# alpc91/SGRL

Measured on AMD Instinct MI355X. Metric: env-steps/sec (whole node) + SET-actor fwd us/step, 3d_walker mix @8192 envs/GPU, higher is better.
Workload: dtype f64 (dynamics) / f32 (SET actor, obs); 1 GPU; 3D_Walker++ 8 variants x 1024 envs per GPU (config 3), random U(-1,1) actions, auto-reset, SET actor forward on every step, random-init weights; envs_per_gpu=8192, obs_max_len=287, action_max_len=21, replay_gather=none (single rank)

## Files before the change

include/sgrl_model.h:

```cpp
#ifndef SGRL_MODEL_H
#define SGRL_MODEL_H

#include <stdint.h>

#ifdef __HIPCC__
#define SGRL_HD __host__ __device__ inline
#else
#define SGRL_HD static inline
#endif

#define SGRL_MAGIC 0x5347524C
#define SGRL_MAXDEPTH 8

enum {
  SGRL_H_MAGIC = 0,
  SGRL_H_NBODY,
  SGRL_H_NJNT,
  SGRL_H_NQ,
  SGRL_H_NV,
  SGRL_H_NU,
  SGRL_H_NGEOM,
  SGRL_H_NPAIR,
  SGRL_H_INTEGRATOR,
  SGRL_H_FRAME_SKIP,
  SGRL_H_DONE_RULE,
  SGRL_H_TARGET_V2,
  SGRL_H_RESET_VEL_NORMAL,
  SGRL_H_NHEIGHT_BODIES,
  SGRL_H_HEIGHT_BODY0,
  SGRL_H_HEIGHT_BODY1,
  SGRL_H_MAX_ROWS,
  SGRL_H_PGS_ITERS,
  SGRL_H_SOLVER,
  SGRL_NHDR = 24
};

enum {
  SGRL_F_TIMESTEP = 0,
  SGRL_F_GRAV_X, SGRL_F_GRAV_Y, SGRL_F_GRAV_Z,
  SGRL_F_HEIGHT_LO, SGRL_F_HEIGHT_HI, SGRL_F_ANG_LIMIT,
  SGRL_F_ALIVE_BONUS, SGRL_F_HEADING_WEIGHT, SGRL_F_CTRL_COST,
  SGRL_F_RESET_POS_NOISE, SGRL_F_RESET_VEL_NOISE,
  SGRL_F_PGS_TOL,
  SGRL_F_TOTAL_MASS,
  SGRL_NFHDR = 16
};

enum { SGRL_GEOM_PLANE = 0, SGRL_GEOM_SPHERE = 2, SGRL_GEOM_CAPSULE = 3 };
enum { SGRL_JNT_FREE = 0, SGRL_JNT_HINGE = 3 };

#ifndef SGRL_CONST_AS
#define SGRL_CONST_AS
#endif
#ifndef SGRL_ITAB_AS
#define SGRL_ITAB_AS
#endif
#ifndef SGRL_FTAB_AS
#define SGRL_FTAB_AS
#endif
typedef const SGRL_CONST_AS int32_t* sgrl_hdr_t;
typedef const SGRL_CONST_AS double* sgrl_fhdr_t;
typedef const SGRL_ITAB_AS int32_t* sgrl_itab_t;
typedef const SGRL_FTAB_AS double* sgrl_ftab_t;

typedef struct SgrlModelView {
  sgrl_hdr_t hdr;
  sgrl_fhdr_t fhdr;
  int nbody, njnt, nq, nv, nu, ngeom, npair;
  sgrl_itab_t body_parent, body_jntadr, body_jntnum, body_dofadr, body_dofnum, body_limbtype;
  sgrl_itab_t jnt_type, jnt_body, jnt_qposadr, jnt_dofadr, jnt_limited;
  sgrl_itab_t dof_body, dof_jnt, dof_parent;
  sgrl_itab_t geom_type, geom_body;
  sgrl_itab_t pair_g1, pair_g2, pair_condim;
  sgrl_itab_t act_dof, act_slot;
  sgrl_itab_t body_depth;
  sgrl_itab_t body_path;
  sgrl_itab_t body_subend;
  sgrl_itab_t body_dofmask;
  sgrl_itab_t dof_act;
  sgrl_ftab_t qpos0;
  sgrl_ftab_t body_pos, body_quat, body_ipos, body_inertia, body_mass, body_invweight0;
  sgrl_ftab_t jnt_pos, jnt_axis, jnt_range, jnt_stiffness, jnt_solref, jnt_solimp, jnt_margin;
  sgrl_ftab_t dof_armature, dof_damping, dof_invweight0;
  sgrl_ftab_t geom_pos, geom_quat, geom_size;
  sgrl_ftab_t pair_mu, pair_margin, pair_solref, pair_solimp;
  sgrl_ftab_t act_gear, act_ctrlrange;
  int n_int, n_f64;
} SgrlModelView;

SGRL_HD int sgrl_model_view_dims(const int32_t* dims, sgrl_hdr_t hdr_src, sgrl_fhdr_t fhdr_src, sgrl_itab_t ib, sgrl_ftab_t fb,
                                 SgrlModelView* v) {
  if (dims[SGRL_H_MAGIC] != SGRL_MAGIC) return -1;
  v->hdr = hdr_src;
  v->fhdr = fhdr_src;
  const int nb = dims[SGRL_H_NBODY], nj = dims[SGRL_H_NJNT], nq = dims[SGRL_H_NQ], nv = dims[SGRL_H_NV];
  const int nu = dims[SGRL_H_NU], ng = dims[SGRL_H_NGEOM], np = dims[SGRL_H_NPAIR];
  v->nbody = nb; v->njnt = nj; v->nq = nq; v->nv = nv; v->nu = nu; v->ngeom = ng; v->npair = np;
  sgrl_itab_t p = ib + SGRL_NHDR;
  v->body_parent = p; p += nb;
  v->body_jntadr = p; p += nb;
  v->body_jntnum = p; p += nb;
  v->body_dofadr = p; p += nb;
  v->body_dofnum = p; p += nb;
  v->body_limbtype = p; p += nb;
  v->jnt_type = p; p += nj;
  v->jnt_body = p; p += nj;
  v->jnt_qposadr = p; p += nj;
  v->jnt_dofadr = p; p += nj;
  v->jnt_limited = p; p += nj;
  v->dof_body = p; p += nv;
  v->dof_jnt = p; p += nv;
  v->dof_parent = p; p += nv;
  v->geom_type = p; p += ng;
  v->geom_body = p; p += ng;
  v->pair_g1 = p; p += np;
  v->pair_g2 = p; p += np;
  v->pair_condim = p; p += np;
  v->act_dof = p; p += nu;
  v->act_slot = p; p += nu;
  v->body_depth = p; p += nb;
  v->body_path = p; p += 8 * nb;
  v->body_subend = p; p += nb;
  v->body_dofmask = p; p += 2 * nb;
  v->dof_act = p; p += nv;
  v->n_int = (int)(p - ib);
  sgrl_ftab_t f = fb + SGRL_NFHDR;
  v->qpos0 = f; f += nq;
  v->body_pos = f; f += 3 * nb;
  v->body_quat = f; f += 4 * nb;
  v->body_ipos = f; f += 3 * nb;
  v->body_inertia = f; f += 6 * nb;
  v->body_mass = f; f += nb;
  v->body_invweight0 = f; f += 2 * nb;
  v->jnt_pos = f; f += 3 * nj;
  v->jnt_axis = f; f += 3 * nj;
  v->jnt_range = f; f += 2 * nj;
  v->jnt_stiffness = f; f += nj;
  v->jnt_solref = f; f += 2 * nj;
  v->jnt_solimp = f; f += 5 * nj;
  v->jnt_margin = f; f += nj;
  v->dof_armature = f; f += nv;
  v->dof_damping = f; f += nv;
  v->dof_invweight0 = f; f += nv;
  v->geom_pos = f; f += 3 * ng;
  v->geom_quat = f; f += 4 * ng;
  v->geom_size = f; f += 3 * ng;
  v->pair_mu = f; f += np;
  v->pair_margin = f; f += np;
  v->pair_solref = f; f += 2 * np;
  v->pair_solimp = f; f += 5 * np;
  v->act_gear = f; f += nu;
  v->act_ctrlrange = f; f += 2 * nu;
  v->n_f64 = (int)(f - fb);
  return 0;
}

SGRL_HD int sgrl_model_view_from(sgrl_hdr_t hdr_src, sgrl_fhdr_t fhdr_src, sgrl_itab_t ib, sgrl_ftab_t fb,
                                 SgrlModelView* v) {
  int32_t dims[SGRL_NHDR];
  for (int k = 0; k < SGRL_NHDR; k++) dims[k] = hdr_src[k];
  return sgrl_model_view_dims(dims, hdr_src, fhdr_src, ib, fb, v);
}

SGRL_HD void sgrl_model_blob_sizes(const int32_t* hdr, int* n_int, int* n_f64) {
  const int nb = hdr[SGRL_H_NBODY], nj = hdr[SGRL_H_NJNT], nq = hdr[SGRL_H_NQ], nv = hdr[SGRL_H_NV];
  const int nu = hdr[SGRL_H_NU], ng = hdr[SGRL_H_NGEOM], np = hdr[SGRL_H_NPAIR];
  *n_int = SGRL_NHDR + 18 * nb + 5 * nj + 4 * nv + 2 * ng + 3 * np + 2 * nu;
  *n_f64 = SGRL_NFHDR + nq + 19 * nb + 17 * nj + 3 * nv + 10 * ng + 9 * np + 3 * nu;
}

SGRL_HD int sgrl_model_view(const int32_t* ib, const double* fb, SgrlModelView* v) {
  return sgrl_model_view_from((sgrl_hdr_t)ib, (sgrl_fhdr_t)fb, (sgrl_itab_t)ib, (sgrl_ftab_t)fb, v);
}


#endif
```

sgrl_amd/csrc/engine.hip:

```cpp
#include <hip/hip_runtime.h>

#include <algorithm>
#include <cmath>
#include <cstdio>
#include <cstdlib>
#include <cstring>
#include <string>
#include <vector>

#include "engine_kernel.h"
#include "stream_pick.h"

namespace {

thread_local std::string g_err;

int fail(int code, const std::string& msg) {
  g_err = msg;
  return code;
}
#define HIP_TRY(expr)                                                                              \
  do {                                                                                             \
    hipError_t _e = (expr);                                                                        \
    if (_e != hipSuccess)                                                                          \
// ... 360 lines not shown
  std::vector<int32_t> env_morph;
  std::vector<MorphDev> morphs(n_morph);
  e->d_ib.assign(n_morph, nullptr);
  e->d_fb.assign(n_morph, nullptr);
  int rc = SGRL_OK;
  for (int k = 0; k < n_morph && rc == SGRL_OK; k++) {
    SgrlModelView v;
    if (!ib[k] || !fb[k] || ib_len[k] < SGRL_NHDR || sgrl_model_view(ib[k], fb[k], &v) != 0) { rc = fail(SGRL_ERR_MODEL, "bad magic in model blob " + std::to_string(k)); break; }
    if (v.n_int != ib_len[k] || v.n_f64 != fb_len[k]) { rc = fail(SGRL_ERR_MODEL, "model blob " + std::to_string(k) + " has unexpected length"); break; }
    if (v.nv > 64 || v.nbody > 64 || v.npair > 64) { rc = fail(SGRL_ERR_LIMIT, "morphology exceeds 64 dofs/bodies/pairs"); break; }
    if ((v.nv | 1) > sgrl::kSlabLdy || ib[k][SGRL_H_MAX_ROWS] > sgrl::kSlabRows) { rc = fail(SGRL_ERR_LIMIT, "morphology exceeds the HBM constraint slab (nv <= 46, max_rows <= 256)"); break; }
    e->scratch_stride = std::max(e->scratch_stride, sgrl::slab_doubles(ib[k][SGRL_H_MAX_ROWS], v.nv | 1));
    e->max_geoms = std::max(e->max_geoms, v.ngeom);
    const int L = v.nbody - 1;
    if (41 * L > obs_max_len || 3 * L > action_max_len) { rc = fail(SGRL_ERR_ARG, "obs_max_len/action_max_len too small for morphology " + std::to_string(k)); break; }
    if (morph_count[k] < 0) { rc = fail(SGRL_ERR_ARG, "negative morph_count"); break; }
    sgrl::Layout o;
    sgrl::make_layout(ib[k], &o, v.n_int, SGRL_STAGE_FLOATS ? v.n_f64 : 0);
    if (17 * v.njnt + 7 * v.nbody > (o.lrows + 1) * o.ldy || 6 * v.nv > (o.lrows + 1) * o.ldy) {
      rc = fail(SGRL_ERR_LIMIT, "model " + std::to_string(k) + ": the constraint-row block is too small for the kinematics scratch (17 njnt + 7 nbody doubles)");
      break;
    }
    const int bytes = sgrl::layout_bytes(&o);
    if (bytes > 160 * 1024) { rc = fail(SGRL_ERR_LIMIT, "per-environment LDS slab exceeds 160 KiB"); break; }
    if (bytes > e->lds_bytes) e->lds_bytes = bytes;
    e->morph_lds.push_back(bytes);
    const int need = v.nq + v.nv + 4;
    if (need > e->stride) e->stride = need;
    for (int i = 0; i < morph_count[k]; i++) env_morph.push_back(k);
    if (hipMalloc(&e->d_ib[k], sizeof(int32_t) * ib_len[k]) != hipSuccess || hipMalloc(&e->d_fb[k], sizeof(double) * fb_len[k]) != hipSuccess) { rc = fail(SGRL_ERR_HIP, "hipMalloc(model) failed"); break; }
    (void)hipMemcpy(e->d_ib[k], ib[k], sizeof(int32_t) * ib_len[k], hipMemcpyHostToDevice);
    (void)hipMemcpy(e->d_fb[k], fb[k], sizeof(double) * fb_len[k], hipMemcpyHostToDevice);
    morphs[k].ib = e->d_ib[k];
    morphs[k].fb = e->d_fb[k];
    morphs[k].slot = -1;
    morphs[k].pad_ = 0;
  }
  if (rc == SGRL_OK && env_morph.empty()) rc = fail(SGRL_ERR_ARG, "no environments requested");
  if (rc != SGRL_OK) { sgrl_engine_destroy(e); return rc; }
  e->n_env = (int)env_morph.size();
  e->stride = (e->stride + 1) & ~1;
  bool ok = hipMalloc(&e->d_morphs, sizeof(MorphDev) * n_morph) == hipSuccess &&
            hipMalloc(&e->d_env_morph, sizeof(int32_t) * e->n_env) == hipSuccess &&
            hipMalloc(&e->d_block_env, sizeof(int32_t) * e->n_env) == hipSuccess &&
            hipMalloc(&e->d_step_env, sizeof(int32_t) * e->n_env) == hipSuccess &&
            hipMalloc(&e->d_step_mate, sizeof(int32_t) * e->n_env) == hipSuccess &&
            hipMalloc(&e->d_rec, sizeof(double) * (size_t)e->n_env * e->stride) == hipSuccess &&
            hipMalloc(&e->d_cnt, sizeof(int32_t) * (size_t)e->n_env * 4) == hipSuccess &&
            hipMalloc(&e->d_scratch, sizeof(double) * (size_t)e->n_env * e->scratch_stride) == hipSuccess &&
            hipMalloc(&e->d_cam_dist, sizeof(double) * n_morph) == hipSuccess;
  if (!ok) { sgrl_engine_destroy(e); return fail(SGRL_ERR_HIP, "hipMalloc(state) failed"); }
  e->cam_dist.assign(n_morph, std::nan(""));
  (void)hipMemset(e->d_cam_dist, 0, sizeof(double) * n_morph);
  (void)hipMemcpy(e->d_morphs, morphs.data(), sizeof(MorphDev) * n_morph, hipMemcpyHostToDevice);
  (void)hipMemcpy(e->d_env_morph, env_morph.data(), sizeof(int32_t) * e->n_env, hipMemcpyHostToDevice);
  {
    std::vector<int32_t> order(e->n_env);
    for (int i = 0; i < e->n_env; i++) order[i] = i;
    std::vector<int> spec(n_morph, -1);
    std::vector<int> pair_lds(n_morph, 0);
    std::vector<int> spec_lds(n_morph, 0);
    bool use_specs = false;
    {
      const char* sm = getenv("SGRL_SPECS");
      constexpr int kMaxSpecGroups = 4;
      if (!(sm && sm[0] == '0') && kNumMembers > 0) {
        bool all_light = true, all = true;
        for (int k = 0; k < n_morph; k++) if (morph_count[k] > 0) all_light = all_light && spec_for(ib[k], 4) >= 0;
        const char* pe = getenv("SGRL_PAIR");
        auto pair_bytes = [&](int k) -> int {
          const int m2 = spec_for(ib[k], 2);
          if (m2 < 0 || !kMembers[m2].dims[11] || (pe && pe[0] == '0')) return 0;
          SgrlModelView v;
          (void)sgrl_model_view(ib[k], fb[k], &v);
          sgrl::Layout po;
          sgrl::make_layout(ib[k], &po, v.n_int, 0, true);
          const int pb = sgrl::layout_bytes(&po);
          const bool scratch_ok = 17 * v.njnt + 7 * v.nbody <= (po.lrows + 1) * po.ldy && 6 * v.nv <= (po.lrows + 1) * po.ldy &&
                                  10 * v.nbody <= (po.lrows + 1) * po.ldy && v.nv <= 15;
          return (sgrl::workgroups_per_cu(pb) >= 8 && scratch_ok) ? pb : 0;
        };
        if (all_light) {
          bool all_pair = true;
          for (int k = 0; k < n_morph; k++) if (morph_count[k] > 0) all_pair = all_pair && morph_count[k] >= 2 && pair_bytes(k) > 0;
          if (all_pair) all_light = false;
        }
        std::vector<int> distinct;
        for (int k = 0; k < n_morph; k++) {
          if (morph_count[k] == 0) continue;
          int mb = spec_for(ib[k], all_light ? 4 : 2);
          all = all && mb >= 0;
          if (mb < 0) continue;
          spec[k] = kMembers[mb].family;
          morphs[k].slot = kMembers[mb].slot;
          spec_lds[k] = e->morph_lds[k];
          if (kFamilies[spec[k]].itab_global) {
            SgrlModelView v;
            (void)sgrl_model_view(ib[k], fb[k], &v);
            sgrl::Layout so;
            sgrl::make_layout(ib[k], &so, 0, SGRL_STAGE_FLOATS ? v.n_f64 : 0);
            if (17 * v.njnt + 7 * v.nbody <= (so.lrows + 1) * so.ldy && 6 * v.nv <= (so.lrows + 1) * so.ldy) spec_lds[k] = sgrl::layout_bytes(&so);
            else all = false;
          }
          if (kMembers[mb].dims[11]) pair_lds[k] = pair_bytes(k);
          if (std::find(distinct.begin(), distinct.end(), spec[k]) == distinct.end()) distinct.push_back(spec[k]);
        }
// ... 275 lines not shown
```

sgrl_amd/csrc/step_body.h:

```cpp
#pragma once

#include <math.h>
#include <stdint.h>

#include "../../include/sgrl_model.h"

#ifdef __HIPCC__
#define SGRL_DEV __device__ __forceinline__
#else
#define SGRL_DEV inline
#endif

namespace sgrl {

constexpr double kMinVal = 1e-15;
constexpr double kMinImp = 0.0001;
constexpr double kMaxImp = 0.9999;
constexpr double kPi = 3.14159265358979323846;
constexpr int kNAMax = 32;
constexpr int kBppMaxIter = 40;
constexpr int kSlabRows = 256;
constexpr int kPivotRows = 64;
constexpr int kPrevRows = 48;
constexpr int kSlabLdy = 47;
// ... 471 lines not shown
      ld6(cd, S + o.cdof + 6 * i);
      inert_mul(buf, ci, cd);
      S[o.L + tri(i) + i] = dot6(cd, buf) + m.dof_armature[i];
      for (int j = m.dof_parent[i]; j >= 0; j = m.dof_parent[j]) {
        double cj[6];
        ld6(cj, S + o.cdof + 6 * j);
        S[o.L + tri(i) + j] = dot6(cj, buf);
      }
    });
    if (W::hdr_const(m, SGRL_H_INTEGRATOR) == 0) {
      if (o.mfull_hbm) {
        double* const mh = big_scratch + slab_rows_doubles(o.maxrows, o.ldy);
        const int nt = nv * (nv + 1) / 2;
        w.lanes(64, [&](int l) { for (int k = l; k < nt; k += 64) mh[k] = S[o.L + k]; });
      } else {
        w.lanes(nv, [&](int i) { for (int k = 0; k <= i; k++) S[o.Mfull + tri(i) + k] = S[o.L + tri(i) + k]; });
      }
    }
    SGRL_TICK(2);
    linv = w.chol_inv_packed(nv, S + o.L, kMinVal);
    if (!linv) cholesky(o.L);
    SGRL_TICK(8);
  }

  SGRL_DEV void cholesky(int base) {
    const int nv = o.nv;
    for (int j = 0; j < nv - 1; j++) {
      double pj = S[base + tri(j) + j];
      if (pj < kMinVal) pj = kMinVal;
      const double wj = 1.0 / pj;
      const int sdim = nv - j - 1;
      w.lanes(sdim * (sdim + 1) / 2, [&](int p) {
        int a, b;
        tri_decode(p, &a, &b);
        const int i = j + 1 + a, k = j + 1 + b;
        S[base + tri(i) + k] -= S[base + tri(i) + j] * S[base + tri(k) + j] * wj;
      });
    }
    w.lanes(nv, [&](int j) {
      double pj = S[base + tri(j) + j];
      if (pj < kMinVal) pj = kMinVal;
      S[o.dinv + j] = sqrt(1.0 / pj);
    });
    w.lanes(nv * (nv - 1) / 2, [&](int p) {
      int a, b;
      tri_decode(p, &a, &b);
      S[base + tri(a + 1) + b] *= S[o.dinv + b];
    });
  }

  SGRL_DEV void solve_upper_inplace(int base, int xo) { w.trsv_upper(o.nv, S + base, S + o.dinv, S + xo); }
  SGRL_DEV void solve_lower_inplace(int base, int xo) { w.trsv_lower(o.nv, S + base, S + o.dinv, S + xo); }

  SGRL_DEV void geom_pose(int g, double* pos, double* mat) {
    const int b = m.geom_body[g];
    double t[3], gp[3], gq[4], gm[9], xm[9];
    ld3(gp, m.geom_pos + 3 * g);
    for (int k = 0; k < 9; k++) xm[k] = S[o.xmat + 9 * b + k];
    mat_vec(t, xm, gp);
    for (int k = 0; k < 3; k++) pos[k] = S[o.xpos + 3 * b + k] + t[k];
    for (int k = 0; k < 4; k++) gq[k] = m.geom_quat[4 * g + k];
    quat2mat(gm, gq);
    for (int r = 0; r < 3; r++)
      for (int c = 0; c < 3; c++) mat[3 * r + c] = xm[3 * r] * gm[c] + xm[3 * r + 1] * gm[3 + c] + xm[3 * r + 2] * gm[6 + c];
  }
  SGRL_DEV void make_frame(double* fr) {
    const double n2 = sqrt(dot3(fr + 3, fr + 3));
    if (n2 < 0.5) {
      fr[3] = 0; fr[4] = 0; fr[5] = 0;
      if (fr[1] < 0.5 && fr[1] > -0.5) fr[4] = 1; else fr[5] = 1;
    }
    const double d = dot3(fr, fr + 3);
    for (int k = 0; k < 3; k++) fr[3 + k] -= d * fr[k];
    const double n = sqrt(dot3(fr + 3, fr + 3));
    if (n < kMinVal) { fr[3] = 1; fr[4] = 0; fr[5] = 0; }
    else for (int k = 0; k < 3; k++) fr[3 + k] /= n;
    cross3(fr + 6, fr, fr + 3);
  }
  SGRL_DEV void put_contact(int slot, bool valid, double dist, const double* pos, const double* normal, const double* tangent) {
    I[o.con_valid + slot] = valid ? 1 : 0;
    if (!valid) return;
    double fr[9];
    for (int k = 0; k < 3; k++) { fr[k] = normal[k]; fr[3 + k] = tangent ? tangent[k] : 0.0; }
    make_frame(fr);
    S[o.con_dist + slot] = dist;
    for (int k = 0; k < 3; k++) S[o.con_pos + 3 * slot + k] = pos[k];
    for (int k = 0; k < 6; k++) S[o.con_frame + o.fstride * slot + k] = fr[k];
  }
  SGRL_DEV void plane_sphere(int slot, double margin, const double* ppos, const double* n, const double* c, double r, const double* tangent) {
    const double d[3] = {c[0] - ppos[0], c[1] - ppos[1], c[2] - ppos[2]};
    const double dist = dot3(d, n) - r;
    double pos[3];
    for (int k = 0; k < 3; k++) pos[k] = c[k] - n[k] * (r + 0.5 * dist);
    put_contact(slot, dist < margin, dist, pos, n, tangent);
  }
  SGRL_DEV void collide() {
    w.lanes(o.np, [&](int p) {
      const int g1 = m.pair_g1[p], g2 = m.pair_g2[p];
      double p1[3], m1[9], p2[3], m2[9];
      geom_pose(g1, p1, m1); geom_pose(g2, p2, m2);
      const double margin = m.pair_margin[p];
      const int t1 = m.geom_type[g1], t2 = m.geom_type[g2];
      if (t1 == SGRL_GEOM_PLANE) {
        const double n[3] = {m1[2], m1[5], m1[8]};
        if (t2 == SGRL_GEOM_SPHERE) {
          plane_sphere(2 * p, margin, p1, n, p2, m.geom_size[3 * g2], nullptr);
          I[o.con_valid + 2 * p + 1] = 0;
        } else {
          const double ax[3] = {m2[2], m2[5], m2[8]};
          const double h = m.geom_size[3 * g2 + 1], r = m.geom_size[3 * g2];
          double ca[3], cb[3];
          for (int k = 0; k < 3; k++) { ca[k] = p2[k] + ax[k] * h; cb[k] = p2[k] - ax[k] * h; }
          plane_sphere(2 * p, margin, p1, n, ca, r, ax);
          plane_sphere(2 * p + 1, margin, p1, n, cb, r, ax);
        }
      } else {
        const double a1[3] = {m1[2], m1[5], m1[8]}, a2[3] = {m2[2], m2[5], m2[8]};
        const double h1 = m.geom_size[3 * g1 + 1], h2 = m.geom_size[3 * g2 + 1];
        const double r1 = m.geom_size[3 * g1], r2 = m.geom_size[3 * g2];
        const double d[3] = {p1[0] - p2[0], p1[1] - p2[1], p1[2] - p2[2]};
        const double bb = dot3(a1, a2), c = dot3(a1, d), f = dot3(a2, d);
        const double den = 1.0 - bb * bb;
        const bool general = fabs(den) >= kMinVal;
        int made = 0;
        I[o.con_valid + 2 * p] = 0;
        I[o.con_valid + 2 * p + 1] = 0;
        for (int q = 0; q < (general ? 1 : 4) && made < 2; q++) {
          double s, t;
          if (general) {
            s = (bb * f - c) / den;
            if (s > h1) s = h1;
            if (s < -h1) s = -h1;
            t = bb * s + f;
            if (t > h2) { t = h2; s = bb * t - c; if (s > h1) s = h1; if (s < -h1) s = -h1; }
            else if (t < -h2) { t = -h2; s = bb * t - c; if (s > h1) s = h1; if (s < -h1) s = -h1; }
          } else if (q < 2) {
            s = q ? -h1 : h1; t = bb * s + f;
            if (t > h2) t = h2;
            if (t < -h2) t = -h2;
          } else {
            t = (q & 1) ? -h2 : h2; s = bb * t - c;
            if (s > h1) s = h1;
            if (s < -h1) s = -h1;
          }
          double c1[3], nn[3];
          for (int k = 0; k < 3; k++) { c1[k] = p1[k] + s * a1[k]; nn[k] = (p2[k] + t * a2[k]) - c1[k]; }
          const double len = sqrt(dot3(nn, nn));
          const double dist = len - r1 - r2;
          if (dist >= margin) continue;
          if (len < kMinVal) { nn[0] = 1; nn[1] = 0; nn[2] = 0; } else for (int k = 0; k < 3; k++) nn[k] /= len;
          double pos[3];
          for (int k = 0; k < 3; k++) pos[k] = c1[k] + nn[k] * (r1 + 0.5 * dist);
          put_contact(2 * p + made, true, dist, pos, nn, nullptr);
          made++;
        }
      }
    });
  }

  SGRL_DEV void bias_and_smooth_force() {
    w.lanes(o.nb, [&](int b) {
      if (b == 0) { for (int k = 0; k < 6; k++) S[o.cfrc + k] = 0; return; }
      double cv[6] = {0, 0, 0, 0, 0, 0};
      double ca[6] = {0, 0, 0, -m.fhdr[SGRL_F_GRAV_X], -m.fhdr[SGRL_F_GRAV_Y], -m.fhdr[SGRL_F_GRAV_Z]};
      const int depth = m.body_depth[b];
      for (int lvl = 0; lvl < depth; lvl++) {
        const int c = m.body_path[8 * b + lvl];
        const int j0 = m.body_jntadr[c], jn = m.body_jntnum[c];
        for (int j = j0; j < j0 + jn; j++) {
          const int d0 = m.jnt_dofadr[j];
// ... 5 lines not shown
            double cd[3][6], dd[6];
            for (int d = 0; d < 3; d++) ld6(cd[d], S + o.cdof + 6 * (d0 + 3 + d));
            for (int d = 0; d < 3; d++) {
              cross_motion(dd, cv, cd[d]);
              const double qv = S[o.qvel + d0 + 3 + d];
              for (int k = 0; k < 6; k++) ca[k] += dd[k] * qv;
            }
            for (int d = 0; d < 3; d++) {
              const double qv = S[o.qvel + d0 + 3 + d];
              for (int k = 0; k < 6; k++) cv[k] += cd[d][k] * qv;
            }
          } else {
            double cd[6], dd[6];
            ld6(cd, S + o.cdof + 6 * d0);
            cross_motion(dd, cv, cd);
            const double qv = S[o.qvel + d0];
            for (int k = 0; k < 6; k++) { ca[k] += dd[k] * qv; cv[k] += cd[k] * qv; }
          }
        }
      }
      double ci[10], f1[6], iv[6], f2[6];
      for (int k = 0; k < 10; k++) ci[k] = S[o.cinert + 10 * b + k];
      inert_mul(f1, ci, ca);
      inert_mul(iv, ci, cv);
      cross_force(f2, cv, iv);
      for (int k = 0; k < 6; k++) S[o.cfrc + 6 * b + k] = f1[k] + f2[k];
    });
    w.lanes(o.nv, [&](int d) {
      const int b = m.dof_body[d], e = m.body_subend[b];
      double f[6] = {0, 0, 0, 0, 0, 0}, cd[6];
      for (int c = b; c < e; c++)
        for (int k = 0; k < 6; k++) f[k] += S[o.cfrc + 6 * c + k];
      ld6(cd, S + o.cdof + 6 * d);
      const double bias = dot6(cd, f);
      const int j = m.dof_jnt[d];
      double passive = -m.dof_damping[d] * S[o.qvel + d];
      if (m.jnt_type[j] == SGRL_JNT_HINGE) {
        const int qa = m.jnt_qposadr[j];
        passive -= m.jnt_stiffness[j] * (S[o.qpos + qa] - m.qpos0[qa]);
      }
      double q = passive - bias;
      const int u = m.dof_act[d];
      if (u >= 0) {
        double c = S[o.ctrl + u];
        const double lo = m.act_ctrlrange[2 * u], hi = m.act_ctrlrange[2 * u + 1];
        if (c < lo) c = lo;
        if (c > hi) c = hi;
        q += m.act_gear[u] * c;
      }
      S[o.qfs + d] = q;
    });
  }

  SGRL_DEV double impedance(const double* solimp, double x_raw) {
    double dmin = solimp[0], dmax = solimp[1], width = solimp[2], mid = solimp[3], power = solimp[4];
    if (dmin < kMinImp) dmin = kMinImp;
    if (dmin > kMaxImp) dmin = kMaxImp;
    if (dmax < kMinImp) dmax = kMinImp;
    if (dmax > kMaxImp) dmax = kMaxImp;
    if (width < 0) width = 0;
    if (mid < kMinImp) mid = kMinImp;
    if (mid > kMaxImp) mid = kMaxImp;
    if (power < 1) power = 1;
    if (dmin == dmax || width <= kMinVal) return 0.5 * (dmin + dmax);
    const double x = fabs(x_raw) / width;
    if (x >= 1) return dmax;
    if (x <= 0) return dmin;
    double y;
    if (power == 1) y = x;
    else if (power == 2) y = (x <= mid) ? (x * x) / mid : 1 - ((1 - x) * (1 - x)) / (1 - mid);
    else if (x <= mid) y = pow(x, power) / pow(mid, power - 1);
    else y = 1 - pow(1 - x, power) / pow(1 - mid, power - 1);
    return dmin + y * (dmax - dmin);
  }
  SGRL_DEV void kb(const double* solref, const double* solimp, double* K, double* B) {
    double dmax = solimp[1];
    if (dmax < kMinImp) dmax = kMinImp;
    if (dmax > kMaxImp) dmax = kMaxImp;
    double tc = solref[0];
    const double dr = solref[1], h2 = 2 * m.fhdr[SGRL_F_TIMESTEP];
    if (tc < h2) tc = h2;
    *K = 1.0 / (dmax * dmax * tc * tc * dr * dr);
    *B = 2.0 / (dmax * tc);
  }

  struct Rows {
    double *Y, *eR, *earef, *eb, *ef, *eidg, *C;
    int32_t *kind, *src, *sub, *flist;
  };
  SGRL_DEV Rows rows_lds() const {
    return Rows{S + o.Y, S + o.eR, S + o.earef, S + o.eb, S + o.ef, S + o.eidg, S + o.dead,
                I + o.row_kind, I + o.row_src, I + o.row_sub, I + o.flist};
  }
  SGRL_DEV Rows rows_hbm() const {
    double* p = big_scratch;
    const int mr = o.maxrows;
    Rows r;
    r.C = p; p += kPivotRows * (kPivotRows + 1) / 2;
    r.Y = p; p += (mr + 1) * o.ldy;
    r.eR = p; p += mr; r.earef = p; p += mr; r.eb = p; p += mr; r.ef = p; p += mr;
    r.eidg = p; p += mr;
    int32_t* q = reinterpret_cast<int32_t*>(p);
    r.kind = q; r.src = q + mr; r.sub = q + 2 * mr; r.flist = q + 3 * mr;
    return r;
  }

  SGRL_DEV int count_rows() {
    const int nitem = 2 * o.nj + o.ncon;
    w.lanes(nitem, [&](int t) {
      int c = 0;
      if (t < 2 * o.nj) {
        const int j = t >> 1, side = (t & 1) ? 1 : -1;
        if (m.jnt_limited[j]) {
          const double q = S[o.qpos + m.jnt_qposadr[j]];
          const double dist = side * (m.jnt_range[2 * j + (side + 1) / 2] - q);
          if (dist < m.jnt_margin[j]) c = 1;
        }
      } else {
        const int sl = t - 2 * o.nj;
        if (I[o.con_valid + sl]) { const int dim = m.pair_condim[sl >> 1]; c = (dim == 1) ? 1 : 2 * (dim - 1); }
      }
      I[o.ecnt + t] = c;
    });
    return (int)w.sum(nitem, [&](int t) { return (double)I[o.ecnt + t]; });
  }

  SGRL_DEV void fill_rows(const Rows& R, int wanted_total, int cap) {
    const int nitem = 2 * o.nj + o.ncon;
    if (wanted_total <= cap) {
      w.lanes(nitem, [&](int t) {
        int pre = 0;
        for (int u = 0; u < t; u++) pre += I[o.ecnt + u];
        const int c = I[o.ecnt + t];
        if (t == 0) { I[o.icnt + IC_NROW_WANTED] = wanted_total; I[o.icnt + IC_NROW] = wanted_total; }
        for (int k = 0; k < c; k++) {
          if (t < 2 * o.nj) { R.kind[pre] = (t & 1) ? ROW_LIMIT_HI : ROW_LIMIT_LO; R.src[pre] = t >> 1; R.sub[pre] = 0; }
          else { R.kind[pre + k] = (c == 1) ? ROW_CON1 : ROW_PYR; R.src[pre + k] = t - 2 * o.nj; R.sub[pre + k] = k; }
        }
      });
      return;
    }
    w.lanes(1, [&](int) {
      int nrow = 0, wanted = 0;
      const int maxrows = cap;
      for (int j = 0; j < o.nj; j++) {
        if (!m.jnt_limited[j]) continue;
        const double q = S[o.qpos + m.jnt_qposadr[j]];
        for (int side = -1; side <= 1; side += 2) {
          const double dist = side * (m.jnt_range[2 * j + (side + 1) / 2] - q);
          if (dist >= m.jnt_margin[j]) continue;
          wanted++;
          if (nrow >= maxrows) continue;
          R.kind[nrow] = side < 0 ? ROW_LIMIT_LO : ROW_LIMIT_HI;
          R.src[nrow] = j; R.sub[nrow] = 0;
          nrow++;
        }
      }
      for (int s = 0; s < o.ncon; s++) {
        if (!I[o.con_valid + s]) continue;
        const int p = s >> 1, dim = m.pair_condim[p];
        const int nr = (dim == 1) ? 1 : 2 * (dim - 1);
        wanted += nr;
        if (nrow + nr > maxrows) continue;
        for (int k = 0; k < nr; k++) {
          R.kind[nrow] = dim == 1 ? ROW_CON1 : ROW_PYR;
          R.src[nrow] = s; R.sub[nrow] = k;
          nrow++;
        }
      }
      I[o.icnt + IC_NROW] = nrow; I[o.icnt + IC_NROW_WANTED] = wanted;
      if (wanted > nrow) I[o.icnt + IC_OVERFLOW] += 1;
    });
  }

  template <bool BIG>
  SGRL_DEV void build_rows_and_halfsolve(const Rows& R) {
    const int nv = o.nv, ldy = o.ldy;
    const int nrow = I[o.icnt + IC_NROW];
    w.lanes(nrow + 1, [&](int r) {
      double* Yr = R.Y + r * ldy;
      if (r == nrow) {
        for (int d = 0; d < nv; d++) Yr[d] = S[o.qfs + d];
        return;
      }
      const int kind = R.kind[r], src = R.src[r], sub = R.sub[r];
      double Rreg, aref;
      if (kind == ROW_LIMIT_LO || kind == ROW_LIMIT_HI) {
        const int j = src, side = kind == ROW_LIMIT_LO ? -1 : 1, dof = m.jnt_dofadr[j];
        for (int d = 0; d < nv; d++) Yr[d] = 0;
        Yr[dof] = -side;
        const double q = S[o.qpos + m.jnt_qposadr[j]];
        const double margin = m.jnt_margin[j];
        const double dist = side * (m.jnt_range[2 * j + (side + 1) / 2] - q);
        double si[5], sr[2], K, B;
        for (int k = 0; k < 5; k++) si[k] = m.jnt_solimp[5 * j + k];
        sr[0] = m.jnt_solref[2 * j]; sr[1] = m.jnt_solref[2 * j + 1];
        const double imp = impedance(si, dist - margin);
        kb(sr, si, &K, &B);
        Rreg = (1 - imp) / imp * m.dof_invweight0[dof];
        if (Rreg < kMinVal) Rreg = kMinVal;
        aref = -B * (-side * S[o.qvel + dof]) - K * imp * (dist - margin);
      } else {
        const int s = src, p = s >> 1;
        const int b1 = m.geom_body[m.pair_g1[p]], b2 = m.geom_body[m.pair_g2[p]];
        const double margin = m.pair_margin[p], dist = S[o.con_dist + s], mu = m.pair_mu[p];
        double off[3], dir[3];
        const double* fr = S + o.con_frame + o.fstride * s;
        for (int k = 0; k < 3; k++) off[k] = S[o.con_pos + 3 * s + k] - S[o.misc + MS_COM + k];
        if (kind == ROW_CON1) {
          for (int k = 0; k < 3; k++) dir[k] = fr[k];
        } else {
          const double sg = (sub & 1) ? -mu : mu;
          double tg[3];
          if (sub >> 1) cross3(tg, fr, fr + 3);
          else ld3(tg, fr + 3);
          for (int k = 0; k < 3; k++) dir[k] = fr[k] + sg * tg[k];
        }
        sgrl_itab_t mk1 = m.body_dofmask + 2 * b1;
        sgrl_itab_t mk2 = m.body_dofmask + 2 * b2;
        double vel = 0;
        for (int d = 0; d < nv; d++) {
          double sgn = 0;
          if (b2 > 0 && dof_in_mask(mk2, d)) sgn += 1.0;
          if (b1 > 0 && dof_in_mask(mk1, d)) sgn -= 1.0;
          double val = 0;
          if (sgn != 0) {
            double cd[6], v[3];
            ld6(cd, S + o.cdof + 6 * d);
            cross3(v, cd, off);
            v[0] += cd[3]; v[1] += cd[4]; v[2] += cd[5];
            val = sgn * dot3(dir, v);
          }
          Yr[d] = val;
          vel += val * S[o.qvel + d];
        }
        double si[5], sr[2], K, B;
        for (int k = 0; k < 5; k++) si[k] = m.pair_solimp[5 * p + k];
        sr[0] = m.pair_solref[2 * p]; sr[1] = m.pair_solref[2 * p + 1];
        const double imp = impedance(si, dist - margin);
        kb(sr, si, &K, &B);
        const double tran = m.body_invweight0[2 * b1] + m.body_invweight0[2 * b2];
        if (kind == ROW_CON1) {
          Rreg = (1 - imp) / imp * tran;
          if (Rreg < kMinVal) Rreg = kMinVal;
        } else {
          double R0 = (1 - imp) / imp * (tran + mu * mu * tran);
          if (R0 < kMinVal) R0 = kMinVal;
          Rreg = 2 * mu * mu * R0;
          if (Rreg < kMinVal) Rreg = kMinVal;
        }
        aref = -B * vel - K * imp * (dist - margin);
      }
      R.eR[r] = Rreg; R.earef[r] = aref;
      const int key = (kind << 16) | (src << 3) | sub;
      double f0 = 0;
      const int pn = I[o.icnt + IC_PREV_N];
      const int pcap = o.prevcap, pl = pn < pcap ? pn : pcap;
      for (int k = 0; k < pl; k++) if (I[o.prev_key + k] == key) f0 = S[o.prev_f + k];
      if (pn > pcap) {
        const double* hf = big_scratch + slab_prev_offset(o.maxrows, o.ldy);
        const int32_t* hk = reinterpret_cast<const int32_t*>(hf + o.maxrows);
        for (int k = pcap; k < pn; k++) if (hk[k] == key) f0 = hf[k];
      }
      R.ef[r] = f0;
    });
    SGRL_TICK(6);
    if (linv) {
      if (BIG || !w.trmm_rows(nrow + 1, nv, S + o.L, R.Y, ldy))
      w.lanes(nrow + 1, [&](int r) {
        double* Yr = R.Y + r * ldy;
        for (int d = nv - 1; d >= 0; d--) {
          const double* Ld = S + o.L + tri(d);
          double s0 = 0, s1 = 0, s2 = 0, s3 = 0;
          int c = 0;
          for (; c + 4 <= d + 1; c += 4) {
            const double a0 = Ld[c], a1 = Ld[c + 1], a2 = Ld[c + 2], a3 = Ld[c + 3];
            const double b0 = Yr[c], b1 = Yr[c + 1], b2 = Yr[c + 2], b3 = Yr[c + 3];
            s0 += a0 * b0; s1 += a1 * b1; s2 += a2 * b2; s3 += a3 * b3;
          }
          for (; c <= d; c++) s0 += Ld[c] * Yr[c];
          Yr[d] = (s0 + s1) + (s2 + s3);
        }
      });
    } else {
      w.trsm_lower_rows(nrow + 1, nv, S + o.L, S + o.dinv, R.Y, ldy);
    }
    SGRL_TICK(9);
    w.lanes(nrow > nv ? nrow : nv, [&](int r) {
      if (r < nrow) {
        const double* Yr = R.Y + r * ldy;
        const double* ys = R.Y + nrow * ldy;
        double q0 = 0, q1 = 0, t0 = 0, t1 = 0;
        int d = 0;
        for (; d + 2 <= nv; d += 2) {
          const double y0 = Yr[d], y1 = Yr[d + 1];
          q0 += y0 * y0; q1 += y1 * y1; t0 += y0 * ys[d]; t1 += y1 * ys[d + 1];
        }
        for (; d < nv; d++) { q0 += Yr[d] * Yr[d]; t0 += Yr[d] * ys[d]; }
        const double Rr = R.eR[r];
        R.eidg[r] = 1.0 / ((q0 + q1) + Rr);
        R.eb[r] = (t0 + t1) - R.earef[r];
      }
      if (r < nv) S[o.vpgs + r] = 0;
    });
  }

  template <bool SMALL, bool CLDS>
  SGRL_DEV bool lcp_block_pivot(const Rows& R, int n, double thresh, int* iters_out) {
    double* const wvp = R.earef;
    double* const xwp = SMALL ? S + o.prev_f : S + o.Y;
    const int nv = o.nv, ldy = o.ldy;
    uint64_t F = w.ballot(n, [&](int i) { return R.ef[i] > 0.0; });
    int patience = 3, best = n + 1;
    for (int iter = 0; iter < kBppMaxIter; iter++) {
      w.fence_lane();
// ... 521 lines not shown
```

sgrl_amd/model_pack.py:

```python
import numpy as np

from . import mjcf
from .env_spec import env_spec_for

NHDR = 24
NFHDR = 16
(H_MAGIC, H_NBODY, H_NJNT, H_NQ, H_NV, H_NU, H_NGEOM, H_NPAIR, H_INTEGRATOR, H_FRAME_SKIP, H_DONE_RULE,
 H_TARGET_V2, H_RESET_VEL_NORMAL, H_NHEIGHT_BODIES, H_HEIGHT_BODY0, H_HEIGHT_BODY1, H_MAX_ROWS,
 H_PGS_ITERS, H_SOLVER) = range(19)
(F_TIMESTEP, F_GRAV_X, F_GRAV_Y, F_GRAV_Z, F_HEIGHT_LO, F_HEIGHT_HI, F_ANG_LIMIT, F_ALIVE_BONUS,
 F_HEADING_WEIGHT, F_CTRL_COST, F_RESET_POS_NOISE, F_RESET_VEL_NOISE, F_PGS_TOL, F_TOTAL_MASS) = range(14)

DEFAULT_MAX_ROWS = 48
DEFAULT_PGS_ITERS = 300
DEFAULT_PGS_TOL = 1e-10
DEFAULT_SOLVER = 1


MAXDEPTH = 8


def _derived_int_tables(model):
    nb, nv = model.nbody, model.nv
    depth = np.zeros(nb, dtype=np.int32)
    path = np.full((nb, MAXDEPTH), -1, dtype=np.int32)
    subend = np.zeros(nb, dtype=np.int32)
    mask = np.zeros((nb, 2), dtype=np.int32)
    for b in range(1, nb):
        chain = []
        a = b
        while a > 0:
            chain.append(a)
            a = int(model.body_parent[a])
        chain.reverse()
        if len(chain) > MAXDEPTH:
            raise ValueError("kinematic chain deeper than %d" % MAXDEPTH)
        depth[b] = len(chain)
        path[b, :len(chain)] = chain
        bits = 0
        for c in chain:
            for d in range(int(model.body_dofadr[c]), int(model.body_dofadr[c]) + int(model.body_dofnum[c])):
                bits |= 1 << d
        lo, hi = bits & 0xFFFFFFFF, (bits >> 32) & 0xFFFFFFFF
        mask[b] = np.array([lo, hi], dtype=np.uint32).view(np.int32)
    for b in range(nb - 1, 0, -1):
        subend[b] = max(subend[b], b + 1)
        p = int(model.body_parent[b])
        if p > 0:
            subend[p] = max(subend[p], subend[b])
    for b in range(1, nb):
        for c in range(b + 1, nb):
            inside = c < subend[b]
            a = c
            anc = False
            while a > 0:
                if a == b:
                    anc = True
                a = int(model.body_parent[a])
            if inside != anc:
                raise ValueError("bodies are not in pre-order")
    if nv > 64:
        raise ValueError("nv > 64 unsupported")
    dof_act = np.full(nv, -1, dtype=np.int32)
    for u in range(model.nu):
        dof_act[int(model.act_dof[u])] = u
    return [depth, path.ravel(), subend, mask.ravel(), dof_act]


def worst_case_rows(model):
    rows = int(np.sum(np.asarray(model.jnt_limited) != 0))
    for k in range(model.npair):
        g2 = int(model.pair_g2[k])
        ncon = 2 if (int(model.geom_type[int(model.pair_g1[k])]) == mjcf.GEOM_PLANE and int(model.geom_type[g2]) == mjcf.GEOM_CAPSULE) else 1
        dim = int(model.pair_condim[k])
        rows += ncon * (1 if dim == 1 else 2 * (dim - 1))
    return rows


def pack_model(model, spec=None, env_name=None, max_rows=DEFAULT_MAX_ROWS, pgs_iters=DEFAULT_PGS_ITERS,
               pgs_tol=DEFAULT_PGS_TOL, solver=DEFAULT_SOLVER):
    if spec is None:
        spec = env_spec_for(env_name or model.name)
    hdr = np.zeros(NHDR, dtype=np.int32)
    hdr[H_MAGIC] = mjcf.MAGIC
    hdr[H_NBODY], hdr[H_NJNT], hdr[H_NQ], hdr[H_NV] = model.nbody, model.njnt, model.nq, model.nv
    hdr[H_NU], hdr[H_NGEOM], hdr[H_NPAIR] = model.nu, model.ngeom, model.npair
    hdr[H_INTEGRATOR] = model.integrator
    hdr[H_FRAME_SKIP] = spec.frame_skip
    hdr[H_DONE_RULE] = spec.done_rule
    hdr[H_TARGET_V2] = 1 if spec.target_v2 else 0
    hdr[H_RESET_VEL_NORMAL] = 1 if spec.reset_vel_normal else 0
    hb = [model.body_names.index(n) for n in spec.height_bodies if n in model.body_names]
    hdr[H_NHEIGHT_BODIES] = len(hb)
    for i, b in enumerate(hb[:2]):
        hdr[H_HEIGHT_BODY0 + i] = b
    hdr[H_MAX_ROWS] = min(int(max_rows), max(1, worst_case_rows(model)))
    hdr[H_PGS_ITERS] = pgs_iters
    hdr[H_SOLVER] = solver
    ints = [hdr]
    for k in mjcf.Model.INT_FIELDS:
        ints.append(np.asarray(getattr(model, k), dtype=np.int32).ravel())
    ints.extend(_derived_int_tables(model))
    fh = np.zeros(NFHDR, dtype=np.float64)
    fh[F_TIMESTEP] = model.timestep
    fh[F_GRAV_X:F_GRAV_Z + 1] = model.gravity
    fh[F_HEIGHT_LO], fh[F_HEIGHT_HI], fh[F_ANG_LIMIT] = spec.height_lo, spec.height_hi, spec.ang_limit
    fh[F_ALIVE_BONUS], fh[F_HEADING_WEIGHT], fh[F_CTRL_COST] = spec.alive_bonus, spec.heading_weight, spec.ctrl_cost
    fh[F_RESET_POS_NOISE], fh[F_RESET_VEL_NOISE] = spec.reset_pos_noise, spec.reset_vel_noise
    fh[F_PGS_TOL] = pgs_tol
    fh[F_TOTAL_MASS] = float(np.sum(model.body_mass[1:]))
    fls = [fh]
    for k in mjcf.Model.F64_FIELDS:
        fls.append(np.asarray(getattr(model, k), dtype=np.float64).ravel())
    return np.ascontiguousarray(np.concatenate(ints)), np.ascontiguousarray(np.concatenate(fls))
```

Baseline: 1.998 million env-steps/s.

## Precompute per-row constraint constants and geom axes; ballot-based prefix sums and warm-start lookup

Moves solimp/solref clamping, stiffness/damping (K, B), regularizer factors and geom z-axes into host-side packed model tables, so the device no longer recomputes them per row per step. Geom pose now returns only the axis vector and skips the matrix work for world-attached geoms. Row-count prefix sums use wave ballots and popcounts instead of serial loops when there are 64 items or fewer. Warm-start lookup tries the same row index first and falls back to a linear scan. The model blob grows and the row-count bit packing assumes counts fit in 4 bits. A memset of the record buffer is also added.

After: 2.038 million env-steps/s, median of 6. 1.02x the previous value.

```diff
diff --git a/include/sgrl_model.h b/include/sgrl_model.h
--- a/include/sgrl_model.h
+++ b/include/sgrl_model.h
@@ -46,6 +46,12 @@
   SGRL_NFHDR = 16
 };
 
+enum {
+  SGRL_RC_DMIN = 0, SGRL_RC_DMAX, SGRL_RC_WIDTH, SGRL_RC_MID, SGRL_RC_POWER,
+  SGRL_RC_K, SGRL_RC_B, SGRL_RC_MARGIN, SGRL_RC_MU, SGRL_RC_TRAN, SGRL_RC_RF1, SGRL_RC_RF2,
+  SGRL_ROWC = 12
+};
+
 enum { SGRL_GEOM_PLANE = 0, SGRL_GEOM_SPHERE = 2, SGRL_GEOM_CAPSULE = 3 };
 enum { SGRL_JNT_FREE = 0, SGRL_JNT_HINGE = 3 };
 
@@ -85,6 +91,9 @@
   sgrl_ftab_t geom_pos, geom_quat, geom_size;
   sgrl_ftab_t pair_mu, pair_margin, pair_solref, pair_solimp;
   sgrl_ftab_t act_gear, act_ctrlrange;
+  sgrl_ftab_t geom_axis;
+  sgrl_ftab_t pair_rowc;
+  sgrl_ftab_t jnt_rowc;
   int n_int, n_f64;
 } SgrlModelView;
 
@@ -151,6 +160,9 @@
   v->pair_solimp = f; f += 5 * np;
   v->act_gear = f; f += nu;
   v->act_ctrlrange = f; f += 2 * nu;
+  v->geom_axis = f; f += 3 * ng;
+  v->pair_rowc = f; f += SGRL_ROWC * np;
+  v->jnt_rowc = f; f += SGRL_ROWC * nj;
   v->n_f64 = (int)(f - fb);
   return 0;
 }
@@ -166,7 +178,7 @@
   const int nb = hdr[SGRL_H_NBODY], nj = hdr[SGRL_H_NJNT], nq = hdr[SGRL_H_NQ], nv = hdr[SGRL_H_NV];
   const int nu = hdr[SGRL_H_NU], ng = hdr[SGRL_H_NGEOM], np = hdr[SGRL_H_NPAIR];
   *n_int = SGRL_NHDR + 18 * nb + 5 * nj + 4 * nv + 2 * ng + 3 * np + 2 * nu;
-  *n_f64 = SGRL_NFHDR + nq + 19 * nb + 17 * nj + 3 * nv + 10 * ng + 9 * np + 3 * nu;
+  *n_f64 = SGRL_NFHDR + nq + 19 * nb + 29 * nj + 3 * nv + 13 * ng + 21 * np + 3 * nu;
 }
 
 SGRL_HD int sgrl_model_view(const int32_t* ib, const double* fb, SgrlModelView* v) {
diff --git a/sgrl_amd/csrc/engine.hip b/sgrl_amd/csrc/engine.hip
--- a/sgrl_amd/csrc/engine.hip
+++ b/sgrl_amd/csrc/engine.hip
@@ -436,6 +436,7 @@
   if (!ok) { sgrl_engine_destroy(e); return fail(SGRL_ERR_HIP, "hipMalloc(state) failed"); }
   e->cam_dist.assign(n_morph, std::nan(""));
   (void)hipMemset(e->d_cam_dist, 0, sizeof(double) * n_morph);
+  (void)hipMemset(e->d_rec, 0, sizeof(double) * (size_t)e->n_env * e->stride);
   (void)hipMemcpy(e->d_morphs, morphs.data(), sizeof(MorphDev) * n_morph, hipMemcpyHostToDevice);
   (void)hipMemcpy(e->d_env_morph, env_morph.data(), sizeof(int32_t) * e->n_env, hipMemcpyHostToDevice);
   {
diff --git a/sgrl_amd/csrc/step_body.h b/sgrl_amd/csrc/step_body.h
--- a/sgrl_amd/csrc/step_body.h
+++ b/sgrl_amd/csrc/step_body.h
@@ -547,17 +547,20 @@
   SGRL_DEV void solve_upper_inplace(int base, int xo) { w.trsv_upper(o.nv, S + base, S + o.dinv, S + xo); }
   SGRL_DEV void solve_lower_inplace(int base, int xo) { w.trsv_lower(o.nv, S + base, S + o.dinv, S + xo); }
 
-  SGRL_DEV void geom_pose(int g, double* pos, double* mat) {
+  SGRL_DEV void geom_pose(int g, double* pos, double* ax) {
     const int b = m.geom_body[g];
-    double t[3], gp[3], gq[4], gm[9], xm[9];
+    double gp[3], ga[3];
     ld3(gp, m.geom_pos + 3 * g);
+    ld3(ga, m.geom_axis + 3 * g);
+    if (b == 0) {
+      for (int k = 0; k < 3; k++) { pos[k] = gp[k]; ax[k] = ga[k]; }
+      return;
+    }
+    double t[3], xm[9];
     for (int k = 0; k < 9; k++) xm[k] = S[o.xmat + 9 * b + k];
     mat_vec(t, xm, gp);
     for (int k = 0; k < 3; k++) pos[k] = S[o.xpos + 3 * b + k] + t[k];
-    for (int k = 0; k < 4; k++) gq[k] = m.geom_quat[4 * g + k];
-    quat2mat(gm, gq);
-    for (int r = 0; r < 3; r++)
-      for (int c = 0; c < 3; c++) mat[3 * r + c] = xm[3 * r] * gm[c] + xm[3 * r + 1] * gm[3 + c] + xm[3 * r + 2] * gm[6 + c];
+    mat_vec(ax, xm, ga);
   }
   SGRL_DEV void make_frame(double* fr) {
     const double n2 = sqrt(dot3(fr + 3, fr + 3));
@@ -592,17 +595,17 @@
   SGRL_DEV void collide() {
     w.lanes(o.np, [&](int p) {
       const int g1 = m.pair_g1[p], g2 = m.pair_g2[p];
-      double p1[3], m1[9], p2[3], m2[9];
-      geom_pose(g1, p1, m1); geom_pose(g2, p2, m2);
+      double p1[3], a1[3], p2[3], a2[3];
+      geom_pose(g1, p1, a1); geom_pose(g2, p2, a2);
       const double margin = m.pair_margin[p];
       const int t1 = m.geom_type[g1], t2 = m.geom_type[g2];
       if (t1 == SGRL_GEOM_PLANE) {
-        const double n[3] = {m1[2], m1[5], m1[8]};
+        const double* n = a1;
         if (t2 == SGRL_GEOM_SPHERE) {
           plane_sphere(2 * p, margin, p1, n, p2, m.geom_size[3 * g2], nullptr);
           I[o.con_valid + 2 * p + 1] = 0;
         } else {
-          const double ax[3] = {m2[2], m2[5], m2[8]};
+          const double* ax = a2;
           const double h = m.geom_size[3 * g2 + 1], r = m.geom_size[3 * g2];
           double ca[3], cb[3];
           for (int k = 0; k < 3; k++) { ca[k] = p2[k] + ax[k] * h; cb[k] = p2[k] - ax[k] * h; }
@@ -610,7 +613,6 @@
           plane_sphere(2 * p + 1, margin, p1, n, cb, r, ax);
         }
       } else {
-        const double a1[3] = {m1[2], m1[5], m1[8]}, a2[3] = {m2[2], m2[5], m2[8]};
         const double h1 = m.geom_size[3 * g1 + 1], h2 = m.geom_size[3 * g2 + 1];
         const double r1 = m.geom_size[3 * g1], r2 = m.geom_size[3 * g2];
         const double d[3] = {p1[0] - p2[0], p1[1] - p2[1], p1[2] - p2[2]};
@@ -722,16 +724,8 @@
     });
   }
 
-  SGRL_DEV double impedance(const double* solimp, double x_raw) {
-    double dmin = solimp[0], dmax = solimp[1], width = solimp[2], mid = solimp[3], power = solimp[4];
-    if (dmin < kMinImp) dmin = kMinImp;
-    if (dmin > kMaxImp) dmin = kMaxImp;
-    if (dmax < kMinImp) dmax = kMinImp;
-    if (dmax > kMaxImp) dmax = kMaxImp;
-    if (width < 0) width = 0;
-    if (mid < kMinImp) mid = kMinImp;
-    if (mid > kMaxImp) mid = kMaxImp;
-    if (power < 1) power = 1;
+  SGRL_DEV double impedance(const double* rc, double x_raw) {
+    const double dmin = rc[SGRL_RC_DMIN], dmax = rc[SGRL_RC_DMAX], width = rc[SGRL_RC_WIDTH], mid = rc[SGRL_RC_MID], power = rc[SGRL_RC_POWER];
     if (dmin == dmax || width <= kMinVal) return 0.5 * (dmin + dmax);
     const double x = fabs(x_raw) / width;
     if (x >= 1) return dmax;
@@ -742,16 +736,6 @@
     else if (x <= mid) y = pow(x, power) / pow(mid, power - 1);
     else y = 1 - pow(1 - x, power) / pow(1 - mid, power - 1);
     return dmin + y * (dmax - dmin);
-  }
-  SGRL_DEV void kb(const double* solref, const double* solimp, double* K, double* B) {
-    double dmax = solimp[1];
-    if (dmax < kMinImp) dmax = kMinImp;
-    if (dmax > kMaxImp) dmax = kMaxImp;
-    double tc = solref[0];
-    const double dr = solref[1], h2 = 2 * m.fhdr[SGRL_F_TIMESTEP];
-    if (tc < h2) tc = h2;
-    *K = 1.0 / (dmax * dmax * tc * tc * dr * dr);
-    *B = 2.0 / (dmax * tc);
   }
 
   struct Rows {
@@ -792,15 +776,29 @@
       }
       I[o.ecnt + t] = c;
     });
+    if (nitem <= 64) {
+      int total = 0;
+      for (int k = 0; k < 4; k++) {
+        cbits[k] = w.ballot(nitem, [&](int t) { return ((I[o.ecnt + t] >> k) & 1) != 0; });
+        total += popcount64(cbits[k]) << k;
+      }
+      return total;
+    }
     return (int)w.sum(nitem, [&](int t) { return (double)I[o.ecnt + t]; });
   }
+  uint64_t cbits[4] = {0, 0, 0, 0};
 
   SGRL_DEV void fill_rows(const Rows& R, int wanted_total, int cap) {
     const int nitem = 2 * o.nj + o.ncon;
     if (wanted_total <= cap) {
       w.lanes(nitem, [&](int t) {
         int pre = 0;
-        for (int u = 0; u < t; u++) pre += I[o.ecnt + u];
+        if (nitem <= 64) {
+          const uint64_t below = (1ull << t) - 1;
+          for (int k = 0; k < 4; k++) pre += popcount64(cbits[k] & below) << k;
+        } else {
+          for (int u = 0; u < t; u++) pre += I[o.ecnt + u];
+        }
         const int c = I[o.ecnt + t];
         if (t == 0) { I[o.icnt + IC_NROW_WANTED] = wanted_total; I[o.icnt + IC_NROW] = wanted_total; }
         for (int k = 0; k < c; k++) {
@@ -854,26 +852,23 @@
         return;
       }
       const int kind = R.kind[r], src = R.src[r], sub = R.sub[r];
-      double Rreg, aref;
-      if (kind == ROW_LIMIT_LO || kind == ROW_LIMIT_HI) {
+      const bool lim = kind == ROW_LIMIT_LO || kind == ROW_LIMIT_HI;
+      sgrl_ftab_t rcp = lim ? m.jnt_rowc + SGRL_ROWC * src : m.pair_rowc + SGRL_ROWC * (src >> 1);
+      double rc[SGRL_ROWC];
+      for (int k = 0; k < SGRL_ROWC; k++) rc[k] = rcp[k];
+      double dist, vel;
+      if (lim) {
         const int j = src, side = kind == ROW_LIMIT_LO ? -1 : 1, dof = m.jnt_dofadr[j];
         for (int d = 0; d < nv; d++) Yr[d] = 0;
         Yr[dof] = -side;
         const double q = S[o.qpos + m.jnt_qposadr[j]];
-        const double margin = m.jnt_margin[j];
-        const double dist = side * (m.jnt_range[2 * j + (side + 1) / 2] - q);
-        double si[5], sr[2], K, B;
-        for (int k = 0; k < 5; k++) si[k] = m.jnt_solimp[5 * j + k];
-        sr[0] = m.jnt_solref[2 * j]; sr[1] = m.jnt_solref[2 * j + 1];
-        const double imp = impedance(si, dist - margin);
-        kb(sr, si, &K, &B);
-        Rreg = (1 - imp) / imp * m.dof_invweight0[dof];
-        if (Rreg < kMinVal) Rreg = kMinVal;
-        aref = -B * (-side * S[o.qvel + dof]) - K * imp * (dist - margin);
+        dist = side * (m.jnt_range[2 * j + (side + 1) / 2] - q);
+        vel = -side * S[o.qvel + dof];
       } else {
         const int s = src, p = s >> 1;
         const int b1 = m.geom_body[m.pair_g1[p]], b2 = m.geom_body[m.pair_g2[p]];
-        const double margin = m.pair_margin[p], dist = S[o.con_dist + s], mu = m.pair_mu[p];
+        const double mu = rc[SGRL_RC_MU];
+        dist = S[o.con_dist + s];
         double off[3], dir[3];
         const double* fr = S + o.con_frame + o.fstride * s;
         for (int k = 0; k < 3; k++) off[k] = S[o.con_pos + 3 * s + k] - S[o.misc + MS_COM + k];
@@ -888,7 +883,7 @@
         }
         sgrl_itab_t mk1 = m.body_dofmask + 2 * b1;
         sgrl_itab_t mk2 = m.body_dofmask + 2 * b2;
-        double vel = 0;
+        vel = 0;
         for (int d = 0; d < nv; d++) {
           double sgn = 0;
           if (b2 > 0 && dof_in_mask(mk2, d)) sgn += 1.0;
@@ -904,33 +899,37 @@
           Yr[d] = val;
           vel += val * S[o.qvel + d];
         }
-        double si[5], sr[2], K, B;
-        for (int k = 0; k < 5; k++) si[k] = m.pair_solimp[5 * p + k];
-        sr[0] = m.pair_solref[2 * p]; sr[1] = m.pair_solref[2 * p + 1];
-        const double imp = impedance(si, dist - margin);
-        kb(sr, si, &K, &B);
-        const double tran = m.body_invweight0[2 * b1] + m.body_invweight0[2 * b2];
-        if (kind == ROW_CON1) {
-          Rreg = (1 - imp) / imp * tran;
-          if (Rreg < kMinVal) Rreg = kMinVal;
-        } else {
-          double R0 = (1 - imp) / imp * (tran + mu * mu * tran);
-          if (R0 < kMinVal) R0 = kMinVal;
-          Rreg = 2 * mu * mu * R0;
-          if (Rreg < kMinVal) Rreg = kMinVal;
-        }
-        aref = -B * vel - K * imp * (dist - margin);
-      }
+      }
+      const bool pyr = kind == ROW_PYR;
+      const double x = dist - rc[SGRL_RC_MARGIN];
+      const double imp = impedance(rc, x);
+      double Rreg = (1 - imp) / imp * (pyr ? rc[SGRL_RC_RF1] : rc[SGRL_RC_TRAN]);
+      if (Rreg < kMinVal) Rreg = kMinVal;
+      if (pyr) {
+        Rreg = rc[SGRL_RC_RF2] * Rreg;
+        if (Rreg < kMinVal) Rreg = kMinVal;
+      }
+      const double aref = -rc[SGRL_RC_B] * vel - rc[SGRL_RC_K] * imp * x;
       R.eR[r] = Rreg; R.earef[r] = aref;
       const int key = (kind << 16) | (src << 3) | sub;
       double f0 = 0;
       const int pn = I[o.icnt + IC_PREV_N];
       const int pcap = o.prevcap, pl = pn < pcap ? pn : pcap;
-      for (int k = 0; k < pl; k++) if (I[o.prev_key + k] == key) f0 = S[o.prev_f + k];
-      if (pn > pcap) {
+      bool hit = false;
+      if (r < pl) {
+        if (I[o.prev_key + r] == key) { f0 = S[o.prev_f + r]; hit = true; }
+      } else if (r < pn) {
         const double* hf = big_scratch + slab_prev_offset(o.maxrows, o.ldy);
         const int32_t* hk = reinterpret_cast<const int32_t*>(hf + o.maxrows);
-        for (int k = pcap; k < pn; k++) if (hk[k] == key) f0 = hf[k];
+        if (hk[r] == key) { f0 = hf[r]; hit = true; }
+      }
+      if (!hit) {
+        for (int k = 0; k < pl; k++) if (I[o.prev_key + k] == key) f0 = S[o.prev_f + k];
+        if (pn > pcap) {
+          const double* hf = big_scratch + slab_prev_offset(o.maxrows, o.ldy);
+          const int32_t* hk = reinterpret_cast<const int32_t*>(hf + o.maxrows);
+          for (int k = pcap; k < pn; k++) if (hk[k] == key) f0 = hf[k];
+        }
       }
       R.ef[r] = f0;
     });
diff --git a/sgrl_amd/model_pack.py b/sgrl_amd/model_pack.py
--- a/sgrl_amd/model_pack.py
+++ b/sgrl_amd/model_pack.py
@@ -67,6 +67,50 @@
     return [depth, path.ravel(), subend, mask.ravel(), dof_act]
 
 
+ROWC = 12
+MIN_IMP, MAX_IMP = 0.0001, 0.9999
+
+
+def _row_constants(solref, solimp, margin, mu, tran, timestep):
+    dmin, dmax, width, mid, power = (float(x) for x in solimp)
+    dmin = min(max(dmin, MIN_IMP), MAX_IMP)
+    dmax = min(max(dmax, MIN_IMP), MAX_IMP)
+    width = max(width, 0.0)
+    mid = min(max(mid, MIN_IMP), MAX_IMP)
+    power = max(power, 1.0)
+    tc, dr = max(float(solref[0]), 2 * float(timestep)), float(solref[1])
+    k = 1.0 / (dmax * dmax * tc * tc * dr * dr)
+    b = 2.0 / (dmax * tc)
+    mu, tran = float(mu), float(tran)
+    return [dmin, dmax, width, mid, power, k, b, float(margin), mu, tran, tran + mu * mu * tran, 2 * mu * mu]
+
+
+def _derived_f64_tables(model):
+    ng, npair, nj = model.ngeom, model.npair, model.njnt
+    gq = np.asarray(model.geom_quat, dtype=np.float64).reshape(ng, 4)
+    axis = np.empty((ng, 3))
+    axis[:, 0] = 2 * (gq[:, 1] * gq[:, 3] + gq[:, 0] * gq[:, 2])
+    axis[:, 1] = 2 * (gq[:, 2] * gq[:, 3] - gq[:, 0] * gq[:, 1])
+    axis[:, 2] = gq[:, 0] * gq[:, 0] - gq[:, 1] * gq[:, 1] - gq[:, 2] * gq[:, 2] + gq[:, 3] * gq[:, 3]
+    iw_body = np.asarray(model.body_invweight0, dtype=np.float64).reshape(-1, 2)
+    iw_dof = np.asarray(model.dof_invweight0, dtype=np.float64).ravel()
+    p_solref = np.asarray(model.pair_solref, dtype=np.float64).reshape(npair, 2)
+    p_solimp = np.asarray(model.pair_solimp, dtype=np.float64).reshape(npair, 5)
+    pair = np.zeros((npair, ROWC))
+    for p in range(npair):
+        b1 = int(model.geom_body[int(model.pair_g1[p])])
+        b2 = int(model.geom_body[int(model.pair_g2[p])])
+        pair[p] = _row_constants(p_solref[p], p_solimp[p], np.ravel(model.pair_margin)[p], np.ravel(model.pair_mu)[p],
+                                 iw_body[b1, 0] + iw_body[b2, 0], model.timestep)
+    j_solref = np.asarray(model.jnt_solref, dtype=np.float64).reshape(nj, 2)
+    j_solimp = np.asarray(model.jnt_solimp, dtype=np.float64).reshape(nj, 5)
+    jnt = np.zeros((nj, ROWC))
+    for j in range(nj):
+        jnt[j] = _row_constants(j_solref[j], j_solimp[j], np.ravel(model.jnt_margin)[j], 0.0,
+                                iw_dof[int(model.jnt_dofadr[j])], model.timestep)
+    return [axis.ravel(), pair.ravel(), jnt.ravel()]
+
+
 def worst_case_rows(model):
     rows = int(np.sum(np.asarray(model.jnt_limited) != 0))
     for k in range(model.npair):
@@ -112,4 +156,5 @@
     fls = [fh]
     for k in mjcf.Model.F64_FIELDS:
         fls.append(np.asarray(getattr(model, k), dtype=np.float64).ravel())
+    fls.extend(_derived_f64_tables(model))
     return np.ascontiguousarray(np.concatenate(ints)), np.ascontiguousarray(np.concatenate(fls))
```
